# BadgerTechnologies/navigation

Measured on AMD Instinct MI355X. Metric: scored trajectories/sec (whole node) + costmap inflation cells/sec, 400x400 map, higher is better.
Workload: dtype f64

## Files before the change

navigation_amd/csrc/navgpu_fleet.h:

```cpp
#pragma once
#include <algorithm>
#include <cfloat>
#include <cmath>
#include <cstdio>
#include <cstdlib>
#include <cstring>
#include <ctime>
#include <mutex>
#include <string>
#include <vector>

#include "navgpu_device.h"

using namespace navgpu;

namespace navgpu {
extern thread_local std::string g_last_error;

#define HIP_TRY(expr)                                                                              \
  do {                                                                                             \
    hipError_t e_ = (expr);                                                                        \
    if (e_ != hipSuccess) {                                                                        \
      g_last_error = std::string(#expr) + ": " + hipGetErrorString(e_);                            \
      return NAVGPU_ERR_HIP;                                                                       \
    }                                                                                              \
  } while (0)

inline hipError_t waitStream(hipStream_t s) { return hipStreamSynchronize(s); }

struct EventPair {
  int kernel;
  hipEvent_t a, b;
};
int ensureCompleteGrids(navgpu_fleet* f, uint32_t first, uint32_t count);
}

struct navgpu_fleet {
  navgpu_fleet_desc desc{};
  std::recursive_mutex mu;
  hipStream_t stream = nullptr;
  CostmapDev cm{};
  PlannerDev pl{};
  bool planner_configured = false, inflation_configured = false, planner_staged = false;
  bool shift_pending = false;
  uint32_t shift_first = 0, shift_count = 0;
  std::vector<void*> allocs;
  std::vector<double> h_origin;
  std::vector<double> h_fp_spec;
  std::vector<uint32_t> h_fp_n;
  navgpu_inflation_params infl{};
  navgpu_obstacle_params obsp{};
  double fp_radius = 0.0;
  std::vector<void*> pinned;
  ObsCsr* hp_obs = nullptr;
  uint32_t *hp_cnt = nullptr, *hp_used = nullptr, *hp_plan_cnt = nullptr;
  float* hp_pts = nullptr;
  double *hp_fpw = nullptr, *hp_pose = nullptr, *hp_plan = nullptr, *hp_front = nullptr;
  int32_t *hp_shift = nullptr, *hp_align = nullptr;
  uint32_t *hp_reach = nullptr, *hp_fpn = nullptr;
  uint8_t *cm_stage_dev = nullptr, *cm_stage_host = nullptr, *pl_stage_dev = nullptr, *pl_stage_host = nullptr;
  size_t cm_stage_bytes = 0, pl_stage_bytes = 0;
  bool bounded_grids = true;
  std::vector<uint8_t> grid_partial;
  std::vector<int32_t> h_box;
  std::vector<uint64_t> inputs_gen, cycle_gen;
  void touchInputs(uint32_t first, uint32_t count) {
    for (uint32_t i = first; i < first + count && i < inputs_gen.size(); ++i) ++inputs_gen[i];
  }
  navgpu_robot_state* hp_state = nullptr;
  navgpu_plan_result* hp_result = nullptr;
  bool hp_dma_pending = false;
  int cycles_in_flight = 1;
  int res_slot = 0;
  hipEvent_t ev_cycle[2] = {nullptr, nullptr}, ev_cm_h2d = nullptr, ev_pl_h2d = nullptr;
  bool ev_cycle_set[2] = {false, false}, ev_cm_set = false, ev_pl_set = false;
  hipError_t waitMirrors(hipEvent_t ev, bool set) {
    if (cycles_in_flight < 2) return navgpu::waitStream(stream);
    return set ? hipEventSynchronize(ev) : hipSuccess;
  }
  struct LocalPlannerState {
    std::vector<double> plan;
    double T[3] = {0, 0, 0};
    bool has_T = false, have_plan = false;
    bool xy_tolerance_latch = false, rotating_to_goal = false;
  };
  std::vector<LocalPlannerState> lp;
  navgpu_local_limits lp_limits{};
  bool lp_configured = false;
  struct TpHost {
    std::vector<double> plan;
    double final_goal_x = 0, final_goal_y = 0;
    bool final_goal_position_valid = false;
    navgpu_tp_state st{};
    std::vector<navgpu_tp_sample> made;
    int n_points = 0;
  };
  TpDev tp{};
  bool tp_configured = false;
  std::vector<TpHost> tph;
  std::vector<double> tp_h_samples, tp_h_start;
  std::vector<TpOut> tp_h_out;
  std::vector<uint32_t> tp_h_nsamples, tp_h_within, tp_h_within_count;
  std::vector<int32_t> tp_h_winner;
  struct FootprintQueries {
    uint32_t cap = 0;
    double *d_poses = nullptr, *d_costs = nullptr, *h_poses = nullptr, *h_costs = nullptr;
    uint32_t *d_off = nullptr, *d_first = nullptr, *h_off = nullptr, *h_first = nullptr;
  } fq;
  struct VoxelExport {
    uint32_t stride = 0;
    uint32_t *d_totals = nullptr, *d_counts = nullptr, *d_obs_counts = nullptr;
// ... 35 lines not shown
      return NAVGPU_ERR_HIP;
    }
    allocs.push_back(q);
    *p = static_cast<T*>(q);
    return NAVGPU_OK;
  }
  template <class T>
  int allocPinned(T** p, size_t count) {
    void* q = nullptr;
    hipError_t e = hipHostMalloc(&q, std::max<size_t>(count * sizeof(T), 16), hipHostMallocDefault);
    if (e != hipSuccess) {
      g_last_error = std::string("hipHostMalloc: ") + hipGetErrorString(e);
      return NAVGPU_ERR_HIP;
    }
    memset(q, 0, std::max<size_t>(count * sizeof(T), 16));
    pinned.push_back(q);
    *p = static_cast<T*>(q);
    return NAVGPU_OK;
  }
  void release(void* q) {
    if (!q) return;
    auto it = std::find(allocs.begin(), allocs.end(), q);
    if (it != allocs.end()) allocs.erase(it);
    hipFree(q);
  }
  void releasePinned(void* q) {
    if (!q) return;
    auto it = std::find(pinned.begin(), pinned.end(), q);
    if (it != pinned.end()) pinned.erase(it);
    hipHostFree(q);
  }
  bool rangeOk(uint32_t first, uint32_t count) const { return count > 0 && first < desc.n_instances && count <= desc.n_instances - first; }

  int beginKernel(int k, EventPair* ep) {
    if (!profiling || !((prof_mask >> k) & 1u)) return NAVGPU_OK;
    if (free_events.empty()) {
      EventPair n{};
      HIP_TRY(hipEventCreate(&n.a));
      HIP_TRY(hipEventCreate(&n.b));
      free_events.push_back(n);
    }
    *ep = free_events.back();
    free_events.pop_back();
    ep->kernel = k;
    HIP_TRY(hipEventRecord(ep->a, stream));
    return NAVGPU_OK;
  }
  int endKernel(EventPair* ep) {
    if (!profiling || !ep->a) return NAVGPU_OK;
    HIP_TRY(hipEventRecord(ep->b, stream));
    events.push_back(*ep);
    if (events.size() > 8192) return foldEvents();
    return NAVGPU_OK;
  }
  int foldEvents() {
    if (events.empty()) return NAVGPU_OK;
    HIP_TRY(waitStream(stream));
    for (auto& e : events) {
      float ms = 0;
      HIP_TRY(hipEventElapsedTime(&ms, e.a, e.b));
      prof_ms[e.kernel] += ms;
      prof_n[e.kernel] += 1;
      free_events.push_back(e);
    }
    events.clear();
    return NAVGPU_OK;
  }
};

#ifndef NAVGPU_TEST_NO_FLEET_LOCK
struct FleetGuard {
  std::lock_guard<std::recursive_mutex> lk;
  explicit FleetGuard(navgpu_fleet* f) : lk(f->mu) { (void)hipSetDevice(f->desc.device); }
};
#else
struct FleetGuard {
  explicit FleetGuard(navgpu_fleet* f) { (void)hipSetDevice(f->desc.device); }
};
#endif

#define PROFILED(fleet, kid, launch_expr)            \
  do {                                               \
    EventPair ep_{};                                 \
    int rc_ = (fleet)->beginKernel((kid), &ep_);     \
    if (rc_) return rc_;                             \
    launch_expr;                                     \
    rc_ = (fleet)->endKernel(&ep_);                  \
    if (rc_) return rc_;                             \
  } while (0)

inline int checkLaunch() {
  hipError_t e = hipGetLastError();
  if (e != hipSuccess) {
    g_last_error = std::string("kernel launch: ") + hipGetErrorString(e);
    return NAVGPU_ERR_HIP;
  }
  return NAVGPU_OK;
}
```

navigation_amd/csrc/navgpu_host.cpp:

```cpp
#include "navgpu_fleet.h"

namespace navgpu {
thread_local std::string g_last_error;
}

extern "C" {

const char* navgpu_version(void) { return "navgpu 0.1 (gfx950)"; }
const char* navgpu_strerror(int status) {
  switch (status) {
    case NAVGPU_OK: return "ok";
    case NAVGPU_ERR_INVALID: return "invalid argument";
    case NAVGPU_ERR_NO_DEVICE: return "no usable HIP device (this library has no CPU fallback)";
    case NAVGPU_ERR_HIP: return "HIP runtime error";
    case NAVGPU_ERR_CAPACITY: return "input exceeds a capacity given at fleet creation";
    case NAVGPU_ERR_STATE: return "call sequence violated";
    default: return "unknown status";
  }
}
const char* navgpu_last_error(void) { return g_last_error.c_str(); }
int navgpu_device_count(void) {
  int n = 0;
  if (hipGetDeviceCount(&n) != hipSuccess) return 0;
  return n;
// ... 204 lines not shown
  f->grid_partial.assign(n, 0);
  f->obs_consumed.assign(n, 0);
  f->bounded_grids = true;
  f->h_box.assign((size_t)n * 4, 0);
  f->inputs_gen.assign(n, 0);
  f->cycle_gen.assign(n, 0);
  launch_fill_u8(cm.master, cm.master_default, (size_t)n * cm.cells_padded, f->stream);
  if (cm.obst) launch_fill_u8(cm.obst, cm.obstacle_default, (size_t)n * cm.cells_padded, f->stream);
  if (cm.voxel) launch_fill_u32(cm.voxel, 0x0000FFFFu, (size_t)n * cm.cells_padded, f->stream);
  std::vector<InstCostmapState> st(n);
  for (auto& s : st) {
    memset(&s, 0, sizeof(s));
    s.last_min_x = -FLT_MAX;
    s.last_min_y = -FLT_MAX;
    s.last_max_x = FLT_MAX;
    s.last_max_y = FLT_MAX;
  }
  hipError_t e = hipMemcpyAsync(cm.state, st.data(), sizeof(InstCostmapState) * n, hipMemcpyHostToDevice, f->stream);
  if (e == hipSuccess) e = hipMemsetAsync(pl.bfs_reach, 0, sizeof(uint32_t) * n, f->stream);
  if (e == hipSuccess) e = hipMemsetAsync(pl.bfs_levels, 0, sizeof(uint32_t) * 3 * n, f->stream);
  if (e == hipSuccess) e = waitStream(f->stream);
  if (e != hipSuccess || checkLaunch() != NAVGPU_OK) {
    if (e != hipSuccess) g_last_error = std::string("fleet init: ") + hipGetErrorString(e);
    navgpu_fleet_destroy(f);
    return NAVGPU_ERR_NO_DEVICE;
  }
  *out = f;
  return NAVGPU_OK;
}

int navgpu_fleet_destroy(navgpu_fleet* f) {
  if (!f) return NAVGPU_ERR_INVALID;
  if (f->stream) waitStream(f->stream);
  for (auto& e : f->events) {
    hipEventDestroy(e.a);
    hipEventDestroy(e.b);
  }
  for (auto& e : f->free_events) {
    hipEventDestroy(e.a);
    hipEventDestroy(e.b);
  }
  for (hipEvent_t e : {f->ev_cycle[0], f->ev_cycle[1], f->ev_cm_h2d, f->ev_pl_h2d})
    if (e) hipEventDestroy(e);
  for (void* p : f->allocs) hipFree(p);
  for (void* p : f->pinned) hipHostFree(p);
  if (f->stream) hipStreamDestroy(f->stream);
  delete f;
  return NAVGPU_OK;
}
int navgpu_sync(navgpu_fleet* f) {
  if (!f) return NAVGPU_ERR_INVALID;
  FleetGuard guard_(f);
  HIP_TRY(waitStream(f->stream));
  return NAVGPU_OK;
}
void* navgpu_stream(navgpu_fleet* f) { return f ? (void*)f->stream : nullptr; }
int navgpu_fleet_set_alloc_limit(navgpu_fleet* f, uint64_t max_bytes) {
  if (!f) return NAVGPU_ERR_INVALID;
  FleetGuard guard_(f);
  f->alloc_limit = (size_t)max_bytes;
  return NAVGPU_OK;
}

int navgpu_fleet_set_origin(navgpu_fleet* f, uint32_t first, uint32_t count, const double* xy) {
  if (!f || !xy || !f->rangeOk(first, count)) return NAVGPU_ERR_INVALID;
  FleetGuard guard_(f);
  f->touchInputs(first, count);
  memcpy(&f->h_origin[(size_t)first * 2], xy, sizeof(double) * 2 * count);
  HIP_TRY(hipMemcpyAsync(f->cm.origin + (size_t)first * 2, xy, sizeof(double) * 2 * count, hipMemcpyHostToDevice, f->stream));
  HIP_TRY(waitStream(f->stream));
  return NAVGPU_OK;
}

int navgpu_fleet_get_origin(navgpu_fleet* f, uint32_t first, uint32_t count, double* xy) {
  if (!f || !xy || !f->rangeOk(first, count)) return NAVGPU_ERR_INVALID;
  FleetGuard guard_(f);
  memcpy(xy, &f->h_origin[(size_t)first * 2], sizeof(double) * 2 * count);
  return NAVGPU_OK;
}

static int gridInfo(navgpu_fleet* f, int grid, void** base, size_t* elem, size_t* stride_elems, size_t* used_elems) {
  CostmapDev& cm = f->cm;
  PlannerDev& pl = f->pl;
  switch (grid) {
    case NAVGPU_GRID_MASTER: *base = cm.master; *elem = 1; *stride_elems = cm.cells_padded; break;
    case NAVGPU_GRID_STATIC: *base = cm.stat; *elem = 1; *stride_elems = cm.cells_padded; break;
// ... 464 lines not shown
  uint32_t stride = f->pl.prep_stride;
  if (f->planner_configured) {
    planWindow(f, np, fp_n, fp_spec, fp_radius);
    int rc = allocPrep(f, np, &fresh_prep, &stride);
    if (rc != NAVGPU_OK) return rc;
  }
  hipError_t e = waitStream(f->stream);
  if (e == hipSuccess)
    e = hipMemcpyAsync(f->pl.fp_spec + (size_t)first * kMaxFootprint * 2, &fp_spec[(size_t)first * kMaxFootprint * 2], sizeof(double) * kMaxFootprint * 2 * count,
                       hipMemcpyHostToDevice, f->stream);
  if (e == hipSuccess) e = hipMemcpyAsync(f->pl.fp_n + first, &fp_n[first], sizeof(uint32_t) * count, hipMemcpyHostToDevice, f->stream);
  if (e == hipSuccess) e = waitStream(f->stream);
  if (e != hipSuccess) {
    if (fresh_prep) f->release(fresh_prep);
    g_last_error = std::string("navgpu_set_footprint: ") + hipGetErrorString(e);
    return NAVGPU_ERR_HIP;
  }
  f->h_fp_n.swap(fp_n);
  f->h_fp_spec.swap(fp_spec);
  f->fp_radius = fp_radius;
  if (f->planner_configured) {
    uint8_t* keep = fresh_prep ? fresh_prep : f->pl.prep;
    if (fresh_prep) f->release(f->pl.prep);
    f->pl = np;
    f->pl.prep = keep;
    f->pl.prep_stride = stride;
  }
  return NAVGPU_OK;
}

int navgpu_costmap_stage(navgpu_fleet* f, uint32_t first, uint32_t count, const double* poses, const navgpu_observation* obs,
                         uint32_t n_obs, const float* points, uint32_t n_points_total) {
  if (!f || !poses || !f->rangeOk(first, count) || (n_obs && (!obs || (!points && n_points_total)))) return NAVGPU_ERR_INVALID;
  FleetGuard guard_(f);
  CostmapDev& cm = f->cm;
  if (f->desc.rolling_window && f->shift_pending) return NAVGPU_ERR_STATE;
  if (f->desc.rolling_window) f->touchInputs(first, count);
  HIP_TRY(f->waitMirrors(f->ev_cm_h2d, f->ev_cm_set));
  for (uint32_t li = 0; li < count; ++li) f->hp_cnt[first + li] = f->hp_used[first + li] = 0;
  std::fill(f->obs_consumed.begin() + first, f->obs_consumed.begin() + first + count, 0);
  for (uint32_t k = 0; k < n_obs; ++k) {
    const navgpu_observation& o = obs[k];
    if (o.instance < first || o.instance >= first + count) return NAVGPU_ERR_INVALID;
    const uint32_t i = o.instance;
    if (f->hp_cnt[i] >= cm.max_obs || f->hp_used[i] + o.n_points > cm.max_points) return NAVGPU_ERR_CAPACITY;
    if ((uint64_t)o.first_point + o.n_points > n_points_total) return NAVGPU_ERR_INVALID;
    ObsCsr& d = f->hp_obs[(size_t)i * cm.max_obs + f->hp_cnt[i]++];
    d.first_point = f->hp_used[i];
    d.n_points = o.n_points;
    d.flags = o.flags;
    d.pad = 0;
    d.ox = o.origin_x;
    d.oy = o.origin_y;
    d.oz = o.origin_z;
    d.obstacle_range = o.obstacle_range;
    d.raytrace_range = o.raytrace_range;
    if (o.n_points)
      memcpy(&f->hp_pts[((size_t)i * cm.max_points + f->hp_used[i]) * 3], points + (size_t)o.first_point * 3, sizeof(float) * 3 * o.n_points);
    f->hp_used[i] += o.n_points;
  }
  if (f->desc.rolling_window) {
    const double size_m_x = (cm.nx - 1 + 0.5) * cm.res, size_m_y = (cm.ny - 1 + 0.5) * cm.res;
    for (uint32_t li = 0; li < count; ++li) {
      double& ox = f->h_origin[(size_t)(first + li) * 2];
      double& oy = f->h_origin[(size_t)(first + li) * 2 + 1];
      const double new_origin_x = poses[3 * li] - size_m_x / 2, new_origin_y = poses[3 * li + 1] - size_m_y / 2;
      const int cell_ox = int((new_origin_x - ox) / cm.res), cell_oy = int((new_origin_y - oy) / cm.res);
      ox = ox + cell_ox * cm.res;
      oy = oy + cell_oy * cm.res;
      f->hp_shift[2 * (first + li)] = cell_ox;
      f->hp_shift[2 * (first + li) + 1] = cell_oy;
    }
    HIP_TRY(hipMemcpyAsync(cm.shift + (size_t)first * 2, f->hp_shift + (size_t)first * 2, sizeof(int32_t) * 2 * count, hipMemcpyHostToDevice, f->stream));
    HIP_TRY(hipMemcpyAsync(cm.origin + (size_t)first * 2, &f->h_origin[(size_t)first * 2], sizeof(double) * 2 * count, hipMemcpyHostToDevice, f->stream));
    f->shift_pending = true;
    f->shift_first = first;
    f->shift_count = count;
  }
  for (uint32_t li = 0; li < count; ++li) {
    const uint32_t i = first + li;
    const double x = poses[3 * li], y = poses[3 * li + 1], th = poses[3 * li + 2];
    f->hp_pose[3 * i] = x;
    f->hp_pose[3 * i + 1] = y;
    f->hp_pose[3 * i + 2] = th;
    const double cos_th = cos(th), sin_th = sin(th);
    for (uint32_t v = 0; v < f->h_fp_n[i]; ++v) {
      const double sx = f->h_fp_spec[((size_t)i * kMaxFootprint + v) * 2], sy = f->h_fp_spec[((size_t)i * kMaxFootprint + v) * 2 + 1];
      f->hp_fpw[((size_t)i * kMaxFootprint + v) * 2] = x + (sx * cos_th - sy * sin_th);
      f->hp_fpw[((size_t)i * kMaxFootprint + v) * 2 + 1] = y + (sx * sin_th + sy * cos_th);
    }
  }
  memcpy(f->hp_fpn + first, &f->h_fp_n[first], sizeof(uint32_t) * count);
  if (first == 0 && count == f->desc.n_instances) {
    HIP_TRY(hipMemcpyAsync(f->cm_stage_dev, f->cm_stage_host, f->cm_stage_bytes, hipMemcpyHostToDevice, f->stream));
  } else {
    HIP_TRY(hipMemcpyAsync(cm.pose + (size_t)first * 3, f->hp_pose + (size_t)first * 3, sizeof(double) * 3 * count, hipMemcpyHostToDevice, f->stream));
    HIP_TRY(hipMemcpyAsync(cm.obs + (size_t)first * cm.max_obs, f->hp_obs + (size_t)first * cm.max_obs, sizeof(ObsCsr) * (size_t)count * cm.max_obs, hipMemcpyHostToDevice, f->stream));
    HIP_TRY(hipMemcpyAsync(cm.obs_count + first, f->hp_cnt + first, sizeof(uint32_t) * count, hipMemcpyHostToDevice, f->stream));
    HIP_TRY(hipMemcpyAsync(cm.points + (size_t)first * cm.max_points * 3, f->hp_pts + (size_t)first * cm.max_points * 3, sizeof(float) * 3 * (size_t)count * cm.max_points, hipMemcpyHostToDevice, f->stream));
    HIP_TRY(hipMemcpyAsync(cm.fp_world + (size_t)first * kMaxFootprint * 2, f->hp_fpw + (size_t)first * kMaxFootprint * 2, sizeof(double) * 2 * kMaxFootprint * (size_t)count, hipMemcpyHostToDevice, f->stream));
    HIP_TRY(hipMemcpyAsync(cm.fp_n + first, f->hp_fpn + first, sizeof(uint32_t) * count, hipMemcpyHostToDevice, f->stream));
  }
  if (f->cycles_in_flight > 1) {
    HIP_TRY(hipEventRecord(f->ev_cm_h2d, f->stream));
    f->ev_cm_set = true;
  }
  return NAVGPU_OK;
}

static int applyPendingShift(navgpu_fleet* f, uint32_t first, uint32_t count) {
  CostmapDev& cm = f->cm;
  if (!(f->desc.rolling_window && f->shift_pending)) return NAVGPU_OK;
  if (first != f->shift_first || count != f->shift_count) return NAVGPU_ERR_STATE;
  if (first != 0 || count != f->desc.n_instances) return NAVGPU_ERR_INVALID;
  launch_shift_u8(cm.master, cm.master_alt, cm, first, count, cm.master_default, f->stream);
  std::swap(cm.master, cm.master_alt);
  f->pl.master = cm.master;
  if (cm.obst) {
    launch_shift_u8(cm.obst, cm.obst_alt, cm, first, count, cm.obstacle_default, f->stream);
    std::swap(cm.obst, cm.obst_alt);
  }
  if (cm.voxel) {
    launch_shift_u32(cm.voxel, cm.voxel_alt, cm, first, count, 0x0000FFFFu, f->stream);
    std::swap(cm.voxel, cm.voxel_alt);
  }
  f->shift_pending = false;
  return NAVGPU_OK;
}

int navgpu_costmap_update(navgpu_fleet* f, uint32_t first, uint32_t count) {
  if (!f || !f->rangeOk(first, count)) return NAVGPU_ERR_INVALID;
  FleetGuard guard_(f);
  f->touchInputs(first, count);
  CostmapDev& cm = f->cm;
  if ((cm.layers & NAVGPU_LAYER_INFLATION) && !f->inflation_configured) return NAVGPU_ERR_STATE;
  {
    int rc = applyPendingShift(f, first, count);
    if (rc) return rc;
  }
  PROFILED(f, NAVGPU_K_OBSTACLE, launch_obstacle(cm, first, count, nullptr, 0, f->stream));
  std::fill(f->obs_consumed.begin() + first, f->obs_consumed.begin() + first + count, 1);
  PROFILED(f, NAVGPU_K_MERGE, launch_merge(cm, first, count, nullptr, f->stream));
  if (cm.layers & NAVGPU_LAYER_INFLATION) PROFILED(f, NAVGPU_K_INFLATE, launch_inflate(cm, first, count, nullptr, f->stream));
  return checkLaunch();
}

int navgpu_costmap_bounds(navgpu_fleet* f, uint32_t first, uint32_t count, int32_t* boxes) {
  if (!f || !boxes || !f->rangeOk(first, count)) return NAVGPU_ERR_INVALID;
  FleetGuard guard_(f);
  std::vector<InstCostmapState> st(count);
  HIP_TRY(hipMemcpyAsync(st.data(), f->cm.state + first, sizeof(InstCostmapState) * count, hipMemcpyDeviceToHost, f->stream));
  HIP_TRY(waitStream(f->stream));
  for (uint32_t i = 0; i < count; ++i)
    for (int k = 0; k < 4; ++k) boxes[4 * i + k] = st[i].box[k];
  return NAVGPU_OK;
}

int navgpu_inflate(navgpu_fleet* f, uint32_t first, uint32_t count, const int32_t* boxes) {
  if (!f || !f->rangeOk(first, count)) return NAVGPU_ERR_INVALID;
  FleetGuard guard_(f);
  f->touchInputs(first, count);
  if (!f->inflation_configured) return NAVGPU_ERR_STATE;
  const int32_t* d_boxes = nullptr;
  if (boxes) {
    HIP_TRY(hipMemcpyAsync(f->d_boxes_tmp, boxes, sizeof(int32_t) * 4 * count, hipMemcpyHostToDevice, f->stream));
    d_boxes = f->d_boxes_tmp;
  }
  PROFILED(f, NAVGPU_K_INFLATE, launch_inflate(f->cm, first, count, d_boxes, f->stream));
  if (boxes) HIP_TRY(waitStream(f->stream));
  return checkLaunch();
}

int navgpu_obstacle_update_bounds(navgpu_fleet* f, uint32_t first, uint32_t count, double* bounds) {
  if (!f || !bounds || !f->rangeOk(first, count)) return NAVGPU_ERR_INVALID;
  FleetGuard guard_(f);
  if (!f->cm.obst) return NAVGPU_ERR_STATE;
// ... 203 lines not shown
    f->release(pl.part_cost);
    f->release(pl.part_index);
    f->release(pl.sample_cost);
    f->release(pl.sample_status);
    np.axis_samples = n_axis;
    np.part_cost = n_part_cost;
    np.part_index = n_part_index;
    np.sample_cost = n_sample_cost;
    np.sample_status = n_sample_status;
  }
  if (n_prep) {
    f->release(pl.prep);
    np.prep = n_prep;
    np.prep_stride = n_stride;
  }
  pl = np;
  f->planner_configured = true;
  f->touchInputs(0, nI);
  if ((rc = restageReach(f)) != NAVGPU_OK) return rc;
  HIP_TRY(waitStream(f->stream));
  return NAVGPU_OK;
}

int navgpu_planner_set_plan(navgpu_fleet* f, uint32_t first, uint32_t count) {
  if (!f || !f->rangeOk(first, count)) return NAVGPU_ERR_INVALID;
  FleetGuard guard_(f);
  HIP_TRY(hipMemsetAsync(f->pl.osc_flags + first, 0, sizeof(uint32_t) * count, f->stream));
  return NAVGPU_OK;
}

int navgpu_planner_stage(navgpu_fleet* f, uint32_t first, uint32_t count, const navgpu_robot_state* states, const double* plan_xy,
                         uint32_t n_plan_total) {
  if (!f || !states || !plan_xy || !f->rangeOk(first, count)) return NAVGPU_ERR_INVALID;
  FleetGuard guard_(f);
  if (!f->planner_configured) return NAVGPU_ERR_STATE;
  PlannerDev& pl = f->pl;
  const navgpu_dwa_config& c = pl.cfg;
  for (uint32_t li = 0; li < count; ++li) {
    const navgpu_robot_state& s = states[li];
    if (s.plan_count == 0) return NAVGPU_ERR_INVALID;
    if (s.plan_count > pl.max_plan) return NAVGPU_ERR_CAPACITY;
    if ((uint64_t)s.plan_first + s.plan_count > n_plan_total) return NAVGPU_ERR_INVALID;
  }
  HIP_TRY(f->waitMirrors(f->ev_pl_h2d, f->ev_pl_set));
  for (uint32_t li = 0; li < count; ++li) {
    const uint32_t i = first + li;
    const navgpu_robot_state& s = states[li];
    f->hp_state[i] = s;
    memcpy(&f->hp_plan[(size_t)i * pl.max_plan * 2], plan_xy + (size_t)s.plan_first * 2, sizeof(double) * 2 * s.plan_count);
    f->hp_plan_cnt[i] = s.plan_count;
    const double gx = plan_xy[((size_t)s.plan_first + s.plan_count - 1) * 2], gy = plan_xy[((size_t)s.plan_first + s.plan_count - 1) * 2 + 1];
    const double sq_dist = (s.pos[0] - gx) * (s.pos[0] - gx) + (s.pos[1] - gy) * (s.pos[1] - gy);
    const double angle_to_goal = atan2(gy - s.pos[1], gx - s.pos[0]);
    f->hp_front[2 * i] = gx + c.forward_point_distance * cos(angle_to_goal);
    f->hp_front[2 * i + 1] = gy + c.forward_point_distance * sin(angle_to_goal);
    f->hp_align[i] = sq_dist > c.forward_point_distance * c.forward_point_distance * c.cheat_factor ? 1 : 0;
    f->hp_reach[i] = bfsReachCells(f, s, gx, gy);
  }
  f->touchInputs(first, count);
  if (first == 0 && count == f->desc.n_instances) {
    HIP_TRY(hipMemcpyAsync(f->pl_stage_dev, f->pl_stage_host, f->pl_stage_bytes, hipMemcpyHostToDevice, f->stream));
  } else {
    HIP_TRY(hipMemcpyAsync(pl.state + first, f->hp_state + first, sizeof(navgpu_robot_state) * count, hipMemcpyHostToDevice, f->stream));
    HIP_TRY(hipMemcpyAsync(pl.plan + (size_t)first * pl.max_plan * 2, f->hp_plan + (size_t)first * pl.max_plan * 2, sizeof(double) * 2 * (size_t)count * pl.max_plan, hipMemcpyHostToDevice, f->stream));
    HIP_TRY(hipMemcpyAsync(pl.plan_count + first, f->hp_plan_cnt + first, sizeof(uint32_t) * count, hipMemcpyHostToDevice, f->stream));
    HIP_TRY(hipMemcpyAsync(pl.front_last + (size_t)first * 2, f->hp_front + (size_t)first * 2, sizeof(double) * 2 * count, hipMemcpyHostToDevice, f->stream));
    HIP_TRY(hipMemcpyAsync(pl.align_on + first, f->hp_align + first, sizeof(int32_t) * count, hipMemcpyHostToDevice, f->stream));
    HIP_TRY(hipMemcpyAsync(pl.bfs_reach + first, f->hp_reach + first, sizeof(uint32_t) * count, hipMemcpyHostToDevice, f->stream));
  }
  if (f->cycles_in_flight > 1) {
    HIP_TRY(hipEventRecord(f->ev_pl_h2d, f->stream));
    f->ev_pl_set = true;
  }
  f->planner_staged = true;
  f->hp_dma_pending = true;
  return NAVGPU_OK;
}

int navgpu_planner_stage_poses(navgpu_fleet* f, uint32_t first, uint32_t count, const float* pos_xyth, const float* vel_xyth) {
  if (!f || !pos_xyth || !vel_xyth || !f->rangeOk(first, count)) return NAVGPU_ERR_INVALID;
  FleetGuard guard_(f);
  if (!f->planner_configured || !f->planner_staged) return NAVGPU_ERR_STATE;
  PlannerDev& pl = f->pl;
  const navgpu_dwa_config& c = pl.cfg;
  for (uint32_t i = first; i < first + count; ++i)
    if (!f->hp_plan_cnt[i]) {
      g_last_error = "navgpu_planner_stage_poses: instance " + std::to_string(i) + " has no staged plan";
      return NAVGPU_ERR_STATE;
    }
  if (f->hp_dma_pending) {
    HIP_TRY(f->waitMirrors(f->ev_pl_h2d, f->ev_pl_set));
    f->hp_dma_pending = false;
  }
  for (uint32_t li = 0; li < count; ++li) {
    const uint32_t i = first + li;
    navgpu_robot_state& s = f->hp_state[i];
    for (int k = 0; k < 3; ++k) {
      s.pos[k] = pos_xyth[3 * li + k];
      s.vel[k] = vel_xyth[3 * li + k];
    }
    const double* last = &f->hp_plan[((size_t)i * pl.max_plan + f->hp_plan_cnt[i] - 1) * 2];
    const double gx = last[0], gy = last[1];
    const double sq_dist = (s.pos[0] - gx) * (s.pos[0] - gx) + (s.pos[1] - gy) * (s.pos[1] - gy);
    const double angle_to_goal = atan2(gy - s.pos[1], gx - s.pos[0]);
    f->hp_front[2 * i] = gx + c.forward_point_distance * cos(angle_to_goal);
    f->hp_front[2 * i + 1] = gy + c.forward_point_distance * sin(angle_to_goal);
    f->hp_align[i] = sq_dist > c.forward_point_distance * c.forward_point_distance * c.cheat_factor ? 1 : 0;
    f->hp_reach[i] = bfsReachCells(f, s, gx, gy);
  }
  f->touchInputs(first, count);
  PoseChunk ch;
  ch.state = pl.state;
  ch.front_last = pl.front_last;
  ch.align_on = pl.align_on;
// ... 7 lines not shown
    memcpy(ch.reach, f->hp_reach + ch.first, sizeof(uint32_t) * ch.count);
    launch_stage_poses(ch, f->stream);
  }
  return checkLaunch();
}

int navgpu_planner_wavefront_boxes(navgpu_fleet* f, uint32_t first, uint32_t count, int32_t* boxes) {
  if (!f || !boxes || !f->rangeOk(first, count)) return NAVGPU_ERR_INVALID;
  FleetGuard guard_(f);
  for (uint32_t li = 0; li < count; ++li) {
    const uint32_t i = first + li;
    if (f->grid_partial[i])
      memcpy(boxes + 4 * li, &f->h_box[(size_t)4 * i], sizeof(int32_t) * 4);
    else {
      boxes[4 * li] = 0;
      boxes[4 * li + 1] = (int32_t)f->pl.nx - 1;
      boxes[4 * li + 2] = 0;
      boxes[4 * li + 3] = (int32_t)f->pl.ny - 1;
    }
  }
  return NAVGPU_OK;
}

#ifdef NAVGPU_DEBUG_SWITCHES
extern "C" int navgpu_debug_prep_image(navgpu_fleet* f, uint32_t inst, uint8_t* out, uint32_t cap, uint32_t* win, uint32_t* bytes) {
  waitStream(f->stream);
  const uint32_t n = std::min<uint32_t>(cap, f->pl.prep_stride);
  hipMemcpy(out, f->pl.prep + (size_t)inst * f->pl.prep_stride, n, hipMemcpyDeviceToHost);
  *win = f->pl.win;
  *bytes = n;
  return 0;
}
#endif
int navgpu_planner_cycle(navgpu_fleet* f, uint32_t first, uint32_t count) {
  if (!f || !f->rangeOk(first, count)) return NAVGPU_ERR_INVALID;
  FleetGuard guard_(f);
  if (!f->planner_configured || !f->planner_staged) return NAVGPU_ERR_STATE;
  PlannerDev& pl = f->pl;
  const int prev_slot = f->res_slot;
  if (f->cycles_in_flight > 1) {
    if (first != 0 || count != f->desc.n_instances) return NAVGPU_ERR_STATE;
    pl.result = f->hp_result + (size_t)(prev_slot ^ 1) * f->desc.n_instances;
  }
  pl.bfs_bounded = 1;
  for (uint32_t i = first; i < first + count; ++i) {
    f->grid_partial[i] = robotBox(f, i, f->hp_state[i].pos, f->hp_reach[i], &f->h_box[(size_t)4 * i]) ? 1 : 0;
    f->cycle_gen[i] = f->inputs_gen[i];
  }
  launch_samples(pl, first, count, f->stream);
#ifdef NAVGPU_DEBUG_SWITCHES
  if (getenv("NAVGPU_DEBUG_BFS_TRACE") && !pl.bfs_trace) f->alloc(&pl.bfs_trace, (size_t)f->desc.n_instances * 3 * 8);
#endif
  PROFILED(f, NAVGPU_K_BFS, launch_bfs(pl, first, count, f->stream, pl.bfs_order + (size_t)first * 3, true));
#ifdef NAVGPU_DEBUG_SWITCHES
  if (pl.bfs_trace) {
    std::vector<unsigned long long> h((size_t)count * 24);
    hipMemcpyAsync(h.data(), pl.bfs_trace, h.size() * 8, hipMemcpyDeviceToHost, f->stream);
    waitStream(f->stream);
    if (FILE* fp = fopen(getenv("NAVGPU_DEBUG_BFS_TRACE"), "w")) {
      for (size_t i = 0; i < (size_t)count * 3; ++i)
        fprintf(fp, "%zu %llu %llu %llu %llu %llu %llu %llu %llu\n", i, h[8 * i], h[8 * i + 1] & 0xFFFFFFFFFFFFull, h[8 * i + 1] >> 48, h[8 * i + 2], h[8 * i + 3], h[8 * i + 4], h[8 * i + 5], h[8 * i + 6]);
      fclose(fp);
    }
  }
#endif
  uint32_t n_blocks = 0;
  PROFILED(f, NAVGPU_K_SCORE, n_blocks = launch_score(pl, first, count, nullptr, f->stream));
  PROFILED(f, NAVGPU_K_SELECT, launch_select(pl, first, count, n_blocks, f->stream));
  int rc = checkLaunch();
  if (f->cycles_in_flight > 1) {
    const int slot = prev_slot ^ 1;
    if (rc == NAVGPU_OK && hipEventRecord(f->ev_cycle[slot], f->stream) != hipSuccess) rc = NAVGPU_ERR_HIP;
    if (rc == NAVGPU_OK) {
      f->res_slot = slot;
      f->ev_cycle_set[slot] = true;
    } else {
      pl.result = f->hp_result + (size_t)prev_slot * f->desc.n_instances;
    }
  }
  return rc;
}

int navgpu_planner_set_cycles_in_flight(navgpu_fleet* f, int32_t cycles) {
  if (!f || cycles < 1 || cycles > 2) return NAVGPU_ERR_INVALID;
  FleetGuard guard_(f);
  HIP_TRY(waitStream(f->stream));
  if (cycles > 1)
    for (hipEvent_t* e : {&f->ev_cycle[0], &f->ev_cycle[1], &f->ev_cm_h2d, &f->ev_pl_h2d})
      if (!*e) HIP_TRY(hipEventCreateWithFlags(e, hipEventDisableTiming));
  if (cycles == 1 && f->res_slot) {
    memcpy(f->hp_result, f->hp_result + f->desc.n_instances, sizeof(navgpu_plan_result) * f->desc.n_instances);
    f->res_slot = 0;
    f->pl.result = f->hp_result;
  }
  f->ev_cycle_set[0] = f->ev_cycle_set[1] = f->ev_cm_set = f->ev_pl_set = false;
  f->cycles_in_flight = cycles;
  return NAVGPU_OK;
}

int navgpu_planner_results_previous(navgpu_fleet* f, uint32_t first, uint32_t count, navgpu_plan_result* results) {
  if (!f || !results || !f->rangeOk(first, count)) return NAVGPU_ERR_INVALID;
  FleetGuard guard_(f);
  const int slot = f->res_slot ^ 1;
  if (f->cycles_in_flight < 2 || !f->ev_cycle_set[slot]) return NAVGPU_ERR_STATE;
  HIP_TRY(hipEventSynchronize(f->ev_cycle[slot]));
  memcpy(results, f->hp_result + (size_t)slot * f->desc.n_instances + first, sizeof(navgpu_plan_result) * count);
  return NAVGPU_OK;
}

int navgpu_planner_results(navgpu_fleet* f, uint32_t first, uint32_t count, navgpu_plan_result* results) {
  if (!f || !results || !f->rangeOk(first, count)) return NAVGPU_ERR_INVALID;
  FleetGuard guard_(f);
  HIP_TRY(waitStream(f->stream));
  memcpy(results, f->hp_result + (size_t)f->res_slot * f->desc.n_instances + first, sizeof(navgpu_plan_result) * count);
  return NAVGPU_OK;
}

int navgpu_planner_trajectory(navgpu_fleet* f, uint32_t instance, double* xyth, uint32_t cap) {
  if (!f || !xyth || instance >= f->desc.n_instances) return NAVGPU_ERR_INVALID;
  FleetGuard guard_(f);
  HIP_TRY(waitStream(f->stream));
  const navgpu_plan_result r = f->hp_result[(size_t)f->res_slot * f->desc.n_instances + instance];
  uint32_t n = std::min<uint32_t>(r.n_points > 0 ? r.n_points : 0, cap);
  if (n) {
    HIP_TRY(hipMemcpyAsync(xyth, f->pl.traj + (size_t)instance * f->pl.max_sim_steps * 3, sizeof(double) * 3 * n, hipMemcpyDeviceToHost, f->stream));
    HIP_TRY(waitStream(f->stream));
  }
  return r.n_points;
}

int navgpu_planner_samples(navgpu_fleet* f, uint32_t instance, double* costs, int32_t* status, float* vel, uint32_t cap) {
  if (!f || instance >= f->desc.n_instances) return NAVGPU_ERR_INVALID;
  FleetGuard guard_(f);
  PlannerDev& pl = f->pl;
  if (!pl.sample_cost) return NAVGPU_ERR_STATE;
// ... 143 lines not shown
```

navigation_amd/csrc/planner_score.hip:

```cpp
#include "planner_score.h"

namespace navgpu {

#ifdef NAVGPU_PREP_TIMING
__device__ unsigned long long g_prep_stats[16];
#define PREP_STAMP(i) prep_t[i] = wall_clock64()
#else
#define PREP_STAMP(i)
#endif

struct ScoreRobot {
  uint32_t inst;
  Geom g;
  navgpu_robot_state st;
  const uint8_t* master;
  const uint32_t *dpath, *dgoal, *dfront;
  const int32_t* cnt;
  uint32_t nfp;
  int win, wx0, wy0;
  int win_bytes, nw;
};
__device__ __forceinline__ ScoreRobot scoreRobot(const PlannerDev& pl, uint32_t inst) {
  ScoreRobot r;
  r.inst = inst;
// ... 815 lines not shown
__global__ __launch_bounds__(kScoreThreads) void k_score_explicit(PlannerDev pl, uint32_t first, const float* explicit_sample) {
  scoreExplicit<false>(pl, first, explicit_sample);
}
__global__ __launch_bounds__(kScoreThreads) void k_score_explicit_agg(PlannerDev pl, uint32_t first, const float* explicit_sample) {
  scoreExplicit<true>(pl, first, explicit_sample);
}

size_t score_window_bytes(uint32_t win) {
  return (((size_t)win * win + 15) & ~(size_t)15) + score_bits_bytes((int)win);
}
size_t score_table_row_bytes(const PlannerDev& pl) { return (size_t)pl.tab_steps * ((4 + 2 * pl.tab_nfp) * sizeof(double) + sizeof(float)); }
size_t score_table_bytes(const PlannerDev& pl) {
  return ((size_t)pl.tab_nth * score_table_row_bytes(pl) + 15) & ~(size_t)15;
}
size_t score_table_lds_bytes(const PlannerDev& pl) {
  return ((size_t)pl.tab_rows * score_table_row_bytes(pl) + 15) & ~(size_t)15;
}
uint32_t score_table_rows(const PlannerDev& pl, uint32_t win) {
  const size_t wb = score_window_bytes(win), row = score_table_row_bytes(pl);
  if (row == 0 || wb + score_table_bytes(pl) + score_scratch_bytes((int)win) > 150u * 1024u) return 0;
  for (size_t budget : {(size_t)NAVGPU_SCORE_TAB_LDS_KB * 1024, (size_t)52 * 1024, (size_t)78 * 1024}) {
    if (wb + 16 >= budget) continue;
    const size_t r = (budget - wb - 16) / row;
    if (r >= 1) return (uint32_t)std::min<size_t>(r, pl.tab_nth);
  }
  return 0;
}
size_t score_prep_bytes(const PlannerDev& pl) {
  return score_window_bytes(pl.win) + (pl.use_tables ? score_table_bytes(pl) : 0);
}
size_t score_prep_slot_bytes(const PlannerDev& pl) {
  return ((score_prep_bytes(pl) + 255) & ~(size_t)255) + kScoreAuxBytes + score_prep_reject_bytes(pl);
}
uint32_t launch_score(const PlannerDev& pl_in, uint32_t first, uint32_t count, const float* explicit_sample, hipStream_t s) {
  PlannerDev pl = pl_in;
  const size_t win_bytes = score_window_bytes(pl.win);
  const size_t scratch = score_scratch_bytes((int)pl.win);
  if (explicit_sample) {
    launchScore(pl.mg_generic ? k_score_explicit_agg : k_score_explicit, dim3(1, count), kScoreThreads, win_bytes + scratch, s, pl, first,
                explicit_sample);
    return 1;
  }
  if (score_sweep_applies(pl)) {
    pl.tab_bytes = (uint32_t)score_table_bytes(pl);
    pl.prep_bytes = (uint32_t)score_prep_bytes(pl);
    launchScore(k_score_prep_tab, dim3(1, count), kScorePrepThreads, win_bytes + score_table_bytes(pl) + scratch, s, pl, first);
    return launch_score_sweep(pl, first, count, s);
  }
  pl.use_tables = 0;
  pl.prep_bytes = (uint32_t)score_prep_bytes(pl);
  const uint32_t gen_blocks = (pl.max_samples + kScoreThreads - 1) / kScoreThreads;
  launchScore(k_score_prep_gen, dim3(1, count), kScoreThreads, win_bytes + scratch, s, pl, first);
  auto gen = pl.mg_generic        ? k_score_gen_agg
             : pl.fp_chunk <= 6  ? k_score_gen<6>
             : pl.fp_chunk <= 9  ? k_score_gen<9>
             : pl.fp_chunk <= 12 ? k_score_gen<12>
                                 : k_score_gen<16>;
  launchScore(gen, dim3(gen_blocks, count), kScoreThreads, win_bytes, s, pl, first, explicit_sample);
  return gen_blocks;
}

#ifdef NAVGPU_PREP_TIMING
extern "C" int navgpu_debug_prep_stats(unsigned long long* out16, int reset) {
  if (out16) hipMemcpyFromSymbol(out16, HIP_SYMBOL(g_prep_stats), sizeof(unsigned long long) * 16);
  if (reset) {
    unsigned long long z[16] = {0};
    hipMemcpyToSymbol(HIP_SYMBOL(g_prep_stats), z, sizeof(z));
  }
  return 0;
}
#endif

}
```

Baseline: 5.615 billion.

## Overlap costmap staging and update on a side stream with planner scoring

Adds a second non-blocking HIP stream for costmap stage/update (obstacle, merge, inflate) when the whole fleet is processed with multi-cycle pipelining, gated by events. The planner score path records an event right after the prep kernel copies the costmap window, so the next costmap update can start while the sweep kernel still runs. The aim is to hide costmap work behind scoring. In exchange it adds cross-stream event bookkeeping and depends on a host-side check that the sweep stays inside the copied window. If that ordering reasoning is wrong, results could be corrupted.

```diff
diff --git a/navigation_amd/csrc/navgpu_fleet.h b/navigation_amd/csrc/navgpu_fleet.h
--- a/navigation_amd/csrc/navgpu_fleet.h
+++ b/navigation_amd/csrc/navgpu_fleet.h
@@ -33,6 +33,9 @@
   hipEvent_t a, b;
 };
 int ensureCompleteGrids(navgpu_fleet* f, uint32_t first, uint32_t count);
+__attribute__((weak)) hipError_t streamWaitEvent(hipStream_t s, hipEvent_t e);
+__attribute__((weak)) uint32_t launch_score_marked(const PlannerDev& pl, uint32_t first, uint32_t count, hipStream_t s, hipEvent_t mark, int* marked);
+inline bool sideStreamAvailable() { return streamWaitEvent != nullptr && launch_score_marked != nullptr; }
 }
 
 struct navgpu_fleet {
@@ -77,6 +80,34 @@
   hipError_t waitMirrors(hipEvent_t ev, bool set) {
     if (cycles_in_flight < 2) return navgpu::waitStream(stream);
     return set ? hipEventSynchronize(ev) : hipSuccess;
+  }
+  hipStream_t stream_cm = nullptr;
+  hipEvent_t ev_gate[2] = {nullptr, nullptr}, ev_side[2] = {nullptr, nullptr};
+  int gate_i = 0, side_i = 0;
+  bool side_dirty = false, main_touched = true, prep_gate_set = false, stage_on_side = false;
+  bool sideEligible(uint32_t first, uint32_t count) const {
+    return stream_cm && cycles_in_flight > 1 && first == 0 && count == desc.n_instances && !desc.rolling_window && !(desc.layers & NAVGPU_LAYER_VOXEL);
+  }
+  int joinSide() {
+    if (!side_dirty) return NAVGPU_OK;
+    side_i ^= 1;
+    HIP_TRY(hipEventRecord(ev_side[side_i], stream_cm));
+    HIP_TRY(navgpu::streamWaitEvent(stream, ev_side[side_i]));
+    side_dirty = false;
+    return NAVGPU_OK;
+  }
+  int gateSide(bool use_marker) {
+    if (main_touched || !(use_marker && prep_gate_set)) {
+      gate_i ^= 1;
+      HIP_TRY(hipEventRecord(ev_gate[gate_i], stream));
+    }
+    HIP_TRY(navgpu::streamWaitEvent(stream_cm, ev_gate[gate_i]));
+    main_touched = prep_gate_set = false;
+    return NAVGPU_OK;
+  }
+  int leaveOverlap() {
+    main_touched = true;
+    return joinSide();
   }
   struct LocalPlannerState {
     std::vector<double> plan;
@@ -178,7 +209,7 @@
   }
   bool rangeOk(uint32_t first, uint32_t count) const { return count > 0 && first < desc.n_instances && count <= desc.n_instances - first; }
 
-  int beginKernel(int k, EventPair* ep) {
+  int beginKernel(int k, EventPair* ep, hipStream_t s) {
     if (!profiling || !((prof_mask >> k) & 1u)) return NAVGPU_OK;
     if (free_events.empty()) {
       EventPair n{};
@@ -189,12 +220,12 @@
     *ep = free_events.back();
     free_events.pop_back();
     ep->kernel = k;
-    HIP_TRY(hipEventRecord(ep->a, stream));
-    return NAVGPU_OK;
-  }
-  int endKernel(EventPair* ep) {
+    HIP_TRY(hipEventRecord(ep->a, s));
+    return NAVGPU_OK;
+  }
+  int endKernel(EventPair* ep, hipStream_t s) {
     if (!profiling || !ep->a) return NAVGPU_OK;
-    HIP_TRY(hipEventRecord(ep->b, stream));
+    HIP_TRY(hipEventRecord(ep->b, s));
     events.push_back(*ep);
     if (events.size() > 8192) return foldEvents();
     return NAVGPU_OK;
@@ -202,6 +233,7 @@
   int foldEvents() {
     if (events.empty()) return NAVGPU_OK;
     HIP_TRY(waitStream(stream));
+    if (stream_cm) HIP_TRY(waitStream(stream_cm));
     for (auto& e : events) {
       float ms = 0;
       HIP_TRY(hipEventElapsedTime(&ms, e.a, e.b));
@@ -214,26 +246,34 @@
   }
 };
 
+enum FleetGuardMode { kOneStream, kOverlapped };
 #ifndef NAVGPU_TEST_NO_FLEET_LOCK
 struct FleetGuard {
   std::lock_guard<std::recursive_mutex> lk;
-  explicit FleetGuard(navgpu_fleet* f) : lk(f->mu) { (void)hipSetDevice(f->desc.device); }
+  explicit FleetGuard(navgpu_fleet* f, FleetGuardMode mode = kOneStream) : lk(f->mu) {
+    (void)hipSetDevice(f->desc.device);
+    if (mode == kOneStream) (void)f->leaveOverlap();
+  }
 };
 #else
 struct FleetGuard {
-  explicit FleetGuard(navgpu_fleet* f) { (void)hipSetDevice(f->desc.device); }
+  explicit FleetGuard(navgpu_fleet* f, FleetGuardMode mode = kOneStream) {
+    (void)hipSetDevice(f->desc.device);
+    if (mode == kOneStream) (void)f->leaveOverlap();
+  }
 };
 #endif
 
-#define PROFILED(fleet, kid, launch_expr)            \
-  do {                                               \
-    EventPair ep_{};                                 \
-    int rc_ = (fleet)->beginKernel((kid), &ep_);     \
-    if (rc_) return rc_;                             \
-    launch_expr;                                     \
-    rc_ = (fleet)->endKernel(&ep_);                  \
-    if (rc_) return rc_;                             \
+#define PROFILED_ON(fleet, strm, kid, launch_expr)          \
+  do {                                                      \
+    EventPair ep_{};                                        \
+    int rc_ = (fleet)->beginKernel((kid), &ep_, (strm));    \
+    if (rc_) return rc_;                                    \
+    launch_expr;                                            \
+    rc_ = (fleet)->endKernel(&ep_, (strm));                 \
+    if (rc_) return rc_;                                    \
   } while (0)
+#define PROFILED(fleet, kid, launch_expr) PROFILED_ON(fleet, (fleet)->stream, kid, launch_expr)
 
 inline int checkLaunch() {
   hipError_t e = hipGetLastError();
diff --git a/navigation_amd/csrc/navgpu_host.cpp b/navigation_amd/csrc/navgpu_host.cpp
--- a/navigation_amd/csrc/navgpu_host.cpp
+++ b/navigation_amd/csrc/navgpu_host.cpp
@@ -260,6 +260,7 @@
 int navgpu_fleet_destroy(navgpu_fleet* f) {
   if (!f) return NAVGPU_ERR_INVALID;
   if (f->stream) waitStream(f->stream);
+  if (f->stream_cm) waitStream(f->stream_cm);
   for (auto& e : f->events) {
     hipEventDestroy(e.a);
     hipEventDestroy(e.b);
@@ -268,8 +269,9 @@
     hipEventDestroy(e.a);
     hipEventDestroy(e.b);
   }
-  for (hipEvent_t e : {f->ev_cycle[0], f->ev_cycle[1], f->ev_cm_h2d, f->ev_pl_h2d})
+  for (hipEvent_t e : {f->ev_cycle[0], f->ev_cycle[1], f->ev_cm_h2d, f->ev_pl_h2d, f->ev_gate[0], f->ev_gate[1], f->ev_side[0], f->ev_side[1]})
     if (e) hipEventDestroy(e);
+  if (f->stream_cm) hipStreamDestroy(f->stream_cm);
   for (void* p : f->allocs) hipFree(p);
   for (void* p : f->pinned) hipHostFree(p);
   if (f->stream) hipStreamDestroy(f->stream);
@@ -280,6 +282,7 @@
   if (!f) return NAVGPU_ERR_INVALID;
   FleetGuard guard_(f);
   HIP_TRY(waitStream(f->stream));
+  if (f->stream_cm) HIP_TRY(waitStream(f->stream_cm));
   return NAVGPU_OK;
 }
 void* navgpu_stream(navgpu_fleet* f) { return f ? (void*)f->stream : nullptr; }
@@ -810,8 +813,14 @@
 int navgpu_costmap_stage(navgpu_fleet* f, uint32_t first, uint32_t count, const double* poses, const navgpu_observation* obs,
                          uint32_t n_obs, const float* points, uint32_t n_points_total) {
   if (!f || !poses || !f->rangeOk(first, count) || (n_obs && (!obs || (!points && n_points_total)))) return NAVGPU_ERR_INVALID;
-  FleetGuard guard_(f);
+  FleetGuard guard_(f, kOverlapped);
   CostmapDev& cm = f->cm;
+  const bool side = f->sideEligible(first, count);
+  if (!side) {
+    int rc = f->leaveOverlap();
+    if (rc) return rc;
+  }
+  hipStream_t cs = side ? f->stream_cm : f->stream;
   if (f->desc.rolling_window && f->shift_pending) return NAVGPU_ERR_STATE;
   if (f->desc.rolling_window) f->touchInputs(first, count);
   HIP_TRY(f->waitMirrors(f->ev_cm_h2d, f->ev_cm_set));
@@ -869,8 +878,14 @@
     }
   }
   memcpy(f->hp_fpn + first, &f->h_fp_n[first], sizeof(uint32_t) * count);
+  if (side) {
+    int rc = f->gateSide(true);
+    if (rc) return rc;
+    f->side_dirty = true;
+  }
+  f->stage_on_side = side;
   if (first == 0 && count == f->desc.n_instances) {
-    HIP_TRY(hipMemcpyAsync(f->cm_stage_dev, f->cm_stage_host, f->cm_stage_bytes, hipMemcpyHostToDevice, f->stream));
+    HIP_TRY(hipMemcpyAsync(f->cm_stage_dev, f->cm_stage_host, f->cm_stage_bytes, hipMemcpyHostToDevice, cs));
   } else {
     HIP_TRY(hipMemcpyAsync(cm.pose + (size_t)first * 3, f->hp_pose + (size_t)first * 3, sizeof(double) * 3 * count, hipMemcpyHostToDevice, f->stream));
     HIP_TRY(hipMemcpyAsync(cm.obs + (size_t)first * cm.max_obs, f->hp_obs + (size_t)first * cm.max_obs, sizeof(ObsCsr) * (size_t)count * cm.max_obs, hipMemcpyHostToDevice, f->stream));
@@ -880,7 +895,7 @@
     HIP_TRY(hipMemcpyAsync(cm.fp_n + first, f->hp_fpn + first, sizeof(uint32_t) * count, hipMemcpyHostToDevice, f->stream));
   }
   if (f->cycles_in_flight > 1) {
-    HIP_TRY(hipEventRecord(f->ev_cm_h2d, f->stream));
+    HIP_TRY(hipEventRecord(f->ev_cm_h2d, cs));
     f->ev_cm_set = true;
   }
   return NAVGPU_OK;
@@ -908,7 +923,17 @@
 
 int navgpu_costmap_update(navgpu_fleet* f, uint32_t first, uint32_t count) {
   if (!f || !f->rangeOk(first, count)) return NAVGPU_ERR_INVALID;
-  FleetGuard guard_(f);
+  FleetGuard guard_(f, kOverlapped);
+  const bool side = f->stage_on_side && f->sideEligible(first, count);
+  f->stage_on_side = false;
+  if (!side) {
+    int rc = f->leaveOverlap();
+    if (rc) return rc;
+  } else if (f->main_touched) {
+    int rc = f->gateSide(false);
+    if (rc) return rc;
+  }
+  hipStream_t cs = side ? f->stream_cm : f->stream;
   f->touchInputs(first, count);
   CostmapDev& cm = f->cm;
   if ((cm.layers & NAVGPU_LAYER_INFLATION) && !f->inflation_configured) return NAVGPU_ERR_STATE;
@@ -916,10 +941,11 @@
     int rc = applyPendingShift(f, first, count);
     if (rc) return rc;
   }
-  PROFILED(f, NAVGPU_K_OBSTACLE, launch_obstacle(cm, first, count, nullptr, 0, f->stream));
+  if (side) f->side_dirty = true;
+  PROFILED_ON(f, cs, NAVGPU_K_OBSTACLE, launch_obstacle(cm, first, count, nullptr, 0, cs));
   std::fill(f->obs_consumed.begin() + first, f->obs_consumed.begin() + first + count, 1);
-  PROFILED(f, NAVGPU_K_MERGE, launch_merge(cm, first, count, nullptr, f->stream));
-  if (cm.layers & NAVGPU_LAYER_INFLATION) PROFILED(f, NAVGPU_K_INFLATE, launch_inflate(cm, first, count, nullptr, f->stream));
+  PROFILED_ON(f, cs, NAVGPU_K_MERGE, launch_merge(cm, first, count, nullptr, cs));
+  if (cm.layers & NAVGPU_LAYER_INFLATION) PROFILED_ON(f, cs, NAVGPU_K_INFLATE, launch_inflate(cm, first, count, nullptr, cs));
   return checkLaunch();
 }
 
@@ -1189,7 +1215,7 @@
 int navgpu_planner_stage(navgpu_fleet* f, uint32_t first, uint32_t count, const navgpu_robot_state* states, const double* plan_xy,
                          uint32_t n_plan_total) {
   if (!f || !states || !plan_xy || !f->rangeOk(first, count)) return NAVGPU_ERR_INVALID;
-  FleetGuard guard_(f);
+  FleetGuard guard_(f, kOverlapped);
   if (!f->planner_configured) return NAVGPU_ERR_STATE;
   PlannerDev& pl = f->pl;
   const navgpu_dwa_config& c = pl.cfg;
@@ -1236,7 +1262,7 @@
 
 int navgpu_planner_stage_poses(navgpu_fleet* f, uint32_t first, uint32_t count, const float* pos_xyth, const float* vel_xyth) {
   if (!f || !pos_xyth || !vel_xyth || !f->rangeOk(first, count)) return NAVGPU_ERR_INVALID;
-  FleetGuard guard_(f);
+  FleetGuard guard_(f, kOverlapped);
   if (!f->planner_configured || !f->planner_staged) return NAVGPU_ERR_STATE;
   PlannerDev& pl = f->pl;
   const navgpu_dwa_config& c = pl.cfg;
@@ -1310,10 +1336,30 @@
   return 0;
 }
 #endif
+static bool sweepKeepsToWindow(const navgpu_fleet* f, uint32_t first, uint32_t count) {
+  const PlannerDev& pl = f->pl;
+  const navgpu_dwa_config& c = pl.cfg;
+  if (!pl.use_tables || pl.mg_generic || !(c.max_trans_vel >= 0)) return false;
+  const double vmax = c.max_trans_vel + 1e-4, D = vmax * c.sim_time / pl.res, r = f->fp_radius / pl.res;
+  const double radius = (double)((pl.win - 1) / 2);
+  for (uint32_t i = first; i < first + count; ++i) {
+    const float* pos = f->hp_state[i].pos;
+    const double coord = std::max(fabs((double)pos[0]), fabs((double)pos[1])) + vmax * c.sim_time;
+    const double e = (double)pl.tab_steps * coord * (1.0 / 8388608.0) / pl.res + D * 1e-6;
+    if (!(e <= 1.0) || !(ceil(D + r + e) + 1.0 <= radius)) return false;
+  }
+  return true;
+}
+
 int navgpu_planner_cycle(navgpu_fleet* f, uint32_t first, uint32_t count) {
   if (!f || !f->rangeOk(first, count)) return NAVGPU_ERR_INVALID;
-  FleetGuard guard_(f);
+  FleetGuard guard_(f, kOverlapped);
   if (!f->planner_configured || !f->planner_staged) return NAVGPU_ERR_STATE;
+  {
+    int rc = f->joinSide();
+    if (rc) return rc;
+    f->stage_on_side = false;
+  }
   PlannerDev& pl = f->pl;
   const int prev_slot = f->res_slot;
   if (f->cycles_in_flight > 1) {
@@ -1343,7 +1389,16 @@
   }
 #endif
   uint32_t n_blocks = 0;
-  PROFILED(f, NAVGPU_K_SCORE, n_blocks = launch_score(pl, first, count, nullptr, f->stream));
+  int marked = 0;
+  if (f->sideEligible(first, count) && sweepKeepsToWindow(f, first, count)) {
+    const int gi = f->gate_i ^ 1;
+    PROFILED(f, NAVGPU_K_SCORE, n_blocks = navgpu::launch_score_marked(pl, first, count, f->stream, f->ev_gate[gi], &marked));
+    if (marked) f->gate_i = gi;
+  } else {
+    PROFILED(f, NAVGPU_K_SCORE, n_blocks = launch_score(pl, first, count, nullptr, f->stream));
+  }
+  f->prep_gate_set = marked != 0;
+  if (marked) f->main_touched = false;
   PROFILED(f, NAVGPU_K_SELECT, launch_select(pl, first, count, n_blocks, f->stream));
   int rc = checkLaunch();
   if (f->cycles_in_flight > 1) {
@@ -1366,6 +1421,12 @@
   if (cycles > 1)
     for (hipEvent_t* e : {&f->ev_cycle[0], &f->ev_cycle[1], &f->ev_cm_h2d, &f->ev_pl_h2d})
       if (!*e) HIP_TRY(hipEventCreateWithFlags(e, hipEventDisableTiming));
+  if (cycles > 1 && navgpu::sideStreamAvailable()) {
+    for (hipEvent_t* e : {&f->ev_gate[0], &f->ev_gate[1], &f->ev_side[0], &f->ev_side[1]})
+      if (!*e) HIP_TRY(hipEventCreateWithFlags(e, hipEventDisableTiming));
+    if (!f->stream_cm) HIP_TRY(hipStreamCreateWithFlags(&f->stream_cm, hipStreamNonBlocking));
+  }
+  f->prep_gate_set = f->stage_on_side = false;
   if (cycles == 1 && f->res_slot) {
     memcpy(f->hp_result, f->hp_result + f->desc.n_instances, sizeof(navgpu_plan_result) * f->desc.n_instances);
     f->res_slot = 0;
@@ -1378,7 +1439,7 @@
 
 int navgpu_planner_results_previous(navgpu_fleet* f, uint32_t first, uint32_t count, navgpu_plan_result* results) {
   if (!f || !results || !f->rangeOk(first, count)) return NAVGPU_ERR_INVALID;
-  FleetGuard guard_(f);
+  FleetGuard guard_(f, kOverlapped);
   const int slot = f->res_slot ^ 1;
   if (f->cycles_in_flight < 2 || !f->ev_cycle_set[slot]) return NAVGPU_ERR_STATE;
   HIP_TRY(hipEventSynchronize(f->ev_cycle[slot]));
diff --git a/navigation_amd/csrc/navgpu_side_stream.cpp b/navigation_amd/csrc/navgpu_side_stream.cpp
--- /dev/null
+++ b/navigation_amd/csrc/navgpu_side_stream.cpp
@@ -0,0 +1,5 @@
+#include "navgpu_fleet.h"
+
+namespace navgpu {
+hipError_t streamWaitEvent(hipStream_t s, hipEvent_t e) { return hipStreamWaitEvent(s, e, 0); }
+}
diff --git a/navigation_amd/csrc/planner_score.hip b/navigation_amd/csrc/planner_score.hip
--- a/navigation_amd/csrc/planner_score.hip
+++ b/navigation_amd/csrc/planner_score.hip
@@ -871,8 +871,10 @@
 size_t score_prep_slot_bytes(const PlannerDev& pl) {
   return ((score_prep_bytes(pl) + 255) & ~(size_t)255) + kScoreAuxBytes + score_prep_reject_bytes(pl);
 }
-uint32_t launch_score(const PlannerDev& pl_in, uint32_t first, uint32_t count, const float* explicit_sample, hipStream_t s) {
+static uint32_t launchScoreAt(const PlannerDev& pl_in, uint32_t first, uint32_t count, const float* explicit_sample, hipStream_t s, hipEvent_t mark,
+                              int* marked) {
   PlannerDev pl = pl_in;
+  if (marked) *marked = 0;
   const size_t win_bytes = score_window_bytes(pl.win);
   const size_t scratch = score_scratch_bytes((int)pl.win);
   if (explicit_sample) {
@@ -884,6 +886,7 @@
     pl.tab_bytes = (uint32_t)score_table_bytes(pl);
     pl.prep_bytes = (uint32_t)score_prep_bytes(pl);
     launchScore(k_score_prep_tab, dim3(1, count), kScorePrepThreads, win_bytes + score_table_bytes(pl) + scratch, s, pl, first);
+    if (mark && hipEventRecord(mark, s) == hipSuccess && marked) *marked = 1;
     return launch_score_sweep(pl, first, count, s);
   }
   pl.use_tables = 0;
@@ -899,6 +902,13 @@
   return gen_blocks;
 }
 
+uint32_t launch_score(const PlannerDev& pl, uint32_t first, uint32_t count, const float* explicit_sample, hipStream_t s) {
+  return launchScoreAt(pl, first, count, explicit_sample, s, nullptr, nullptr);
+}
+uint32_t launch_score_marked(const PlannerDev& pl, uint32_t first, uint32_t count, hipStream_t s, hipEvent_t mark, int* marked) {
+  return launchScoreAt(pl, first, count, nullptr, s, mark, marked);
+}
+
 #ifdef NAVGPU_PREP_TIMING
 extern "C" int navgpu_debug_prep_stats(unsigned long long* out16, int reset) {
   if (out16) hipMemcpyFromSymbol(out16, HIP_SYMBOL(g_prep_stats), sizeof(unsigned long long) * 16);
```

Result: slower. 3.506 billion (-37.6%).
